# kylegrover/raymarch-algo-compare

Hardware: AMD Instinct MI355X
Metric: Mrays/sec (mean iters/ray alongside), 1920x1080 Mandelbulb/Standard (higher is better)
Workload: dtype f64

## Files before the change

### include/rm_hip.h

```cpp
#ifndef RM_HIP_H
#define RM_HIP_H

#include <stddef.h>
#include <stdint.h>

#ifdef __cplusplus
extern "C" {
#endif

#define RM_OK 0
#define RM_E_BAD_SCENE (-1)
#define RM_E_BAD_STRATEGY (-2)
#define RM_E_BAD_DIMS (-3)
#define RM_E_NO_DEVICE (-4)
#define RM_E_HIP (-5)
#define RM_E_BAD_ARG (-6)
#define RM_E_RCCL (-7)

#define RM_NUM_SCENES 20
#define RM_NUM_STRATEGIES 11
#define RM_NUM_STRATEGY_KERNELS 13
#define RM_HIST_BINS 544
#define RM_MAX_TIMED 256

// ... 48 lines not shown
    int32_t resume_grid;
    int32_t resume_mode;
    int32_t pipeline;
    int32_t team_grid;
    int32_t queue_first;
    int32_t team_steal;
    int32_t queue_refill_min;
    int32_t queue_retry;
    int32_t team_retry;
    int32_t age_priority;
    int32_t late_teams;
    int32_t exit_backlog;
    int32_t keep_busy;
    int32_t early_handover;
    int32_t early_trips;
    int32_t reserved1;
} RmFrameDesc;

typedef struct RmStats {
    uint64_t total_rays;
    uint64_t hit_count;
    uint64_t sum_iters;
    int32_t iter_max;
    int32_t iter_min;
    uint64_t iter_hist[RM_HIST_BINS];
    uint64_t sum_evals;
} RmStats;

typedef struct RmTiming {
    int32_t warmup;
    int32_t repeats;
// ... 238 lines not shown
```

### raymarch_algo_compare_amd/_native.py

```python
from __future__ import annotations

import ctypes
import os
import threading

import numpy as np

_HERE = os.path.dirname(os.path.abspath(__file__))
LIB_PATH = os.environ.get("RM_HIP_LIB") or os.path.join(_HERE, "librm_hip.so")

RM_NUM_SCENES = 20
RM_NUM_STRATEGIES = 11
RM_NUM_STRATEGY_KERNELS = 13
RM_HIST_BINS = 544
RM_MAX_TIMED = 256

ERROR_NAMES = {0: "RM_OK", -1: "RM_E_BAD_SCENE", -2: "RM_E_BAD_STRATEGY", -3: "RM_E_BAD_DIMS",
               -4: "RM_E_NO_DEVICE", -5: "RM_E_HIP", -6: "RM_E_BAD_ARG", -7: "RM_E_RCCL"}

EXPORTS = [
    "rm_init", "rm_shutdown", "rm_last_error", "rm_device_info", "rm_num_scenes", "rm_num_strategies",
    "rm_default_strategy_params",
    "rm_sdf_eval", "rm_march_rays", "rm_march_rays_team", "rm_render", "rm_render_outputs", "rm_render_device", "rm_stats_device_bytes",
    "rm_read_stats", "rm_bench_device", "rm_alloc_frame", "rm_free_frame", "rm_copy_frame_to_host",
# ... 75 lines not shown
    _fields_ = [("scene_id", ctypes.c_int32), ("strategy_id", ctypes.c_int32),
                ("width", ctypes.c_int32), ("height", ctypes.c_int32),
                ("row0", ctypes.c_int32), ("rows", ctypes.c_int32),
                ("cam", ctypes.c_double * 14), ("march", RmMarchConfig),
                ("tile_rows", ctypes.c_int32), ("refill_min", ctypes.c_int32),
                ("grid_waves", ctypes.c_int32), ("band_rows", ctypes.c_int32),
                ("band_stride", ctypes.c_int32), ("band_offset", ctypes.c_int32),
                ("tile_order_mode", ctypes.c_int32), ("eval_mode", ctypes.c_int32),
                ("suspend_after", ctypes.c_int32 * 2),
                ("resume_grid", ctypes.c_int32), ("resume_mode", ctypes.c_int32),
                ("pipeline", ctypes.c_int32), ("team_grid", ctypes.c_int32), ("queue_first", ctypes.c_int32),
                ("team_steal", ctypes.c_int32), ("queue_refill_min", ctypes.c_int32), ("queue_retry", ctypes.c_int32),
                ("team_retry", ctypes.c_int32), ("age_priority", ctypes.c_int32),
                ("late_teams", ctypes.c_int32), ("exit_backlog", ctypes.c_int32),
                ("keep_busy", ctypes.c_int32), ("early_handover", ctypes.c_int32),
                ("early_trips", ctypes.c_int32), ("reserved1", ctypes.c_int32)]


class RmOutputs(ctypes.Structure):
    _fields_ = [("depth", ctypes.c_void_p), ("iters", ctypes.c_void_p), ("hit", ctypes.c_void_p),
                ("t_raw", ctypes.c_void_p), ("final_sdf", ctypes.c_void_p), ("block_var", ctypes.c_void_p),
                ("evals", ctypes.c_void_p)]


class RmStats(ctypes.Structure):
    _fields_ = [("total_rays", ctypes.c_uint64), ("hit_count", ctypes.c_uint64),
                ("sum_iters", ctypes.c_uint64), ("iter_max", ctypes.c_int32), ("iter_min", ctypes.c_int32),
                ("iter_hist", ctypes.c_uint64 * RM_HIST_BINS), ("sum_evals", ctypes.c_uint64)]


class RmTiming(ctypes.Structure):
# ... 179 lines not shown

def device_info() -> dict:
    L = init()
    info = RmDeviceInfo()
    check(L.rm_device_info(ctypes.byref(info)))
    return {"name": info.name.decode(), "arch": info.arch.decode(), "device_id": info.device_id,
            "compute_units": info.compute_units, "clock_mhz": info.clock_mhz,
            "wavefront_size": info.wavefront_size, "total_mem_bytes": int(info.total_mem_bytes)}


def make_desc(scene_id, strategy_id, cam14, width, height, row0=0, rows=None, max_iterations=512,
              hit_threshold=1e-4, max_distance=100.0, lipschitz=1.0, full=False, tile_rows=0, refill_min=0,
              grid_waves=0, band_rows=0, band_stride=0, band_offset=0, tile_order_mode=0, eval_mode=0,
              suspend_after=(0, 0), resume_grid=0, resume_mode=0, params: dict | None = None, pipeline=0, team_grid=0,
              queue_first=0, team_steal=0, queue_refill_min=0, queue_retry=0, team_retry=0, age_priority=0, late_teams=0,
              exit_backlog=0, keep_busy=0, early_handover=0, early_trips=0) -> RmFrameDesc:
    d = RmFrameDesc()
    d.scene_id, d.strategy_id = int(scene_id), int(strategy_id)
    d.width, d.height = int(width), int(height)
    d.row0 = int(row0)
    d.rows = int(height - row0 if rows is None else rows)
    cam14 = np.asarray(cam14, dtype=np.float64).ravel()
    if cam14.size != 14:
        raise ValueError("cam14 must hold 14 doubles")
    for i in range(14):
        d.cam[i] = float(cam14[i])
    d.march.max_iterations = int(max_iterations)
    d.march.full = 1 if full else 0
    d.march.hit_threshold = float(hit_threshold)
    d.march.max_distance = float(max_distance)
    d.march.lipschitz = float(lipschitz)
    fill_params(d.march, params)
    d.tile_rows, d.refill_min, d.grid_waves = int(tile_rows), int(refill_min), int(grid_waves)
    d.band_rows, d.band_stride, d.band_offset = int(band_rows), int(band_stride), int(band_offset)
    d.tile_order_mode = int(tile_order_mode)
    d.eval_mode = int(eval_mode)
    d.suspend_after[0], d.suspend_after[1] = int(suspend_after[0]), int(suspend_after[1])
    d.resume_grid = int(resume_grid)
    d.resume_mode = int(resume_mode)
    d.pipeline, d.team_grid, d.queue_first, d.team_steal = int(pipeline), int(team_grid), int(queue_first), int(team_steal)
    d.queue_refill_min, d.queue_retry, d.team_retry = int(queue_refill_min), int(queue_retry), int(team_retry)
    d.age_priority = int(age_priority)
    d.late_teams, d.exit_backlog = int(late_teams), int(exit_backlog)
    d.keep_busy = int(keep_busy)
    d.early_handover = int(early_handover)
    d.early_trips = int(early_trips)
    return d


def _ptr(a):
    return None if a is None else a.ctypes.data_as(ctypes.c_void_p)


def _ref(record):
    return ctypes.byref(record) if record is not None else None


def _timing(warmup, repeats):
    if repeats <= 0:
        return None
    tm = RmTiming()
# ... 383 lines not shown
```

### raymarch_algo_compare_amd/csrc/rm_capi.hip

```cpp
#include <hip/hip_runtime.h>
#include <dlfcn.h>
#include <link.h>
#include <rccl/rccl.h>

#include <algorithm>
#include <cstdarg>
#include <cstdio>
#include <cstdlib>
#include <cstring>
#include <map>
#include <memory>
#include <mutex>
#include <optional>
#include <string>
#include <vector>

#include "../../include/rm_hip.h"
#include "rm_kernels.h"
#include "rm_launch_plan.h"
#include "rm_pipeline.h"
#include "rm_scene_program.h"
#include "rm_interval.h"
#include "rm_interval_catalogue.h"
#include "rm_segment.h"
// ... 125 lines not shown
    long long corder_key[12] = { -1 };
    bool corder_valid = false;
    bool pass_timing = false;
    hipEvent_t pev[RM_MAX_PASSES + 1];
    bool pev_ready = false;
    int pass_count = 0;
    bool last_was_pipeline = false;
    const unsigned long long* last_stats = nullptr;
    float long_marks[4] = { 0.f, 0.f, 0.f, 0.f };
    float last_push_ms = 0.f, last_pop_ms = 0.f;
    uint32_t generation = 0;
    struct QueueKey { int stride = 0; int writer = 0; size_t used = 0; } qkey[rm::kQueues];
    hipEvent_t frame_ev = nullptr;
    hipStream_t frame_stream = nullptr;
    bool frame_ev_valid = false;
};

struct State : Session {
    WsBuf stats, depth, iters, hit, traw, fs, bvar, evals, tcost, torder, queue[rm::kQueues];
    WsBuf in[2], out[4];
    WsBuf bstats;
    WsBuf ivprog;
    WsBuf ctl;
    WsBuf busy;
    WsBuf trace, trace_start, trace_detach;
    WsBuf ccost, corder;
    WsBuf ssim_depth, ssim_normal, ssim_color, ssim_hit;
    WsBuf ssim_ref, ssim_part, ssim_ssd, ssim_out;
    WsBuf score_depth, score_normal, score_hit, score_caps;
    WsBuf score_band, score_keys, score_small, score_part;
// ... 218 lines not shown
}

int check_desc(const RmFrameDesc* d)
{
    if (!d) return fail(RM_E_BAD_ARG, "desc is NULL");
    if (int rc = check_scene(d->scene_id)) return rc;
    if (d->strategy_id < 0 || d->strategy_id >= RM_NUM_STRATEGY_KERNELS)
        return fail(RM_E_BAD_STRATEGY, "strategy_id %d out of range", d->strategy_id);
    if (int rc = check_slice(d, d->band_rows > 0 && d->band_stride > 1)) return rc;
    if (d->tile_rows != 0 && d->tile_rows != 4 && d->tile_rows != 1) return fail(RM_E_BAD_ARG, "tile_rows must be 0, 4 or 1");
    if (d->tile_order_mode < 0 || d->tile_order_mode > 4) return fail(RM_E_BAD_ARG, "tile_order_mode must be 0 .. 4");
    if (d->eval_mode < 0 || d->eval_mode > 2) return fail(RM_E_BAD_ARG, "eval_mode must be 0, 1 or 2");
    if (d->resume_mode < 0 || d->resume_mode > 3) return fail(RM_E_BAD_ARG, "resume_mode must be 0..3");
    if (d->resume_grid < 0) return fail(RM_E_BAD_ARG, "negative resume_grid");
    if (d->pipeline < 0 || d->pipeline > 2) return fail(RM_E_BAD_ARG, "pipeline must be 0, 1 or 2");
    if (d->team_grid < 0 || d->queue_first < 0 || d->queue_first > 3 || d->team_steal < 0 || d->team_steal > 2 ||
        d->queue_refill_min < 0 || d->queue_refill_min > 64 || d->queue_retry < 0 || d->team_retry < 0 || d->age_priority < 0)
        return fail(RM_E_BAD_ARG, "bad single-launch tuning field");
    if (d->exit_backlog < 0 || d->late_teams > 65536) return fail(RM_E_BAD_ARG, "bad late-team field");
    if (d->keep_busy > (1 << 20)) return fail(RM_E_BAD_ARG, "keep_busy out of range");
    if (d->early_handover > (1 << 20)) return fail(RM_E_BAD_ARG, "early_handover out of range");
    if (d->early_trips < 0 || d->early_trips > 64) return fail(RM_E_BAD_ARG, "early_trips out of range");
    if (d->band_rows < 0 || d->band_stride < 0 || d->band_offset < 0) return fail(RM_E_BAD_ARG, "negative band parameter");
    if (d->band_rows > 0 && d->band_stride > 1) {
        const int th = d->tile_rows ? d->tile_rows : 4;
        if (d->band_rows % th) return fail(RM_E_BAD_ARG, "band_rows must be a multiple of the tile height %d", th);
        if (d->band_offset >= d->band_stride) return fail(RM_E_BAD_ARG, "band_offset must be < band_stride");
        if (d->rows > 0) {
            const long long y = d->rows - 1;
            const long long last = d->row0 + ((y / d->band_rows) * d->band_stride + d->band_offset) * d->band_rows + y % d->band_rows;
// ... 174 lines not shown
}

int launch_frame(const RmFrameDesc* d, const rm::LaunchPlan& p, rm::KernelArgs a, hipStream_t s);

int launch(const RmFrameDesc* d, const rm::LaunchPlan& p, const rm::KernelArgs& a, hipStream_t s)
{
    if (g.frame_ev_valid && g.frame_stream != s) HIP_TRY(hipStreamWaitEvent(s, g.frame_ev, 0));
    const int rc_frame = launch_frame(d, p, a, s);
    if (rc_frame) return rc_frame;
    if (!g.frame_ev_valid) {
        HIP_TRY(hipEventCreateWithFlags(&g.frame_ev, hipEventDisableTiming));
        g.frame_ev_valid = true;
    }
    HIP_TRY(hipEventRecord(g.frame_ev, s));
    g.frame_stream = s;
    return RM_OK;
}

int launch_frame(const RmFrameDesc* d, const rm::LaunchPlan& p, rm::KernelArgs a, hipStream_t s)
{
    a.raw_outputs = (a.t_raw || a.final_sdf || a.evals) ? 1 : 0;
    const bool own_stats = a.stats == (unsigned long long*)g.stats.p;
    if (!(own_stats && g.stats_ready)) HIP_TRY(hipMemsetAsync(a.stats, 0, kStatsBytes, s));
    if (own_stats) g.stats_ready = a.fused_reduce != 0;
    if (d->rows == 0) return RM_OK;
    if (p.refuse) return fail(RM_E_BAD_ARG, "%s", p.refuse);
    const rm::SceneLaunchers* const sc = launchers(d->scene_id);
    const int ntiles = a.tiles_per_frame * a.nframes;
    int order = p.tile_order;
    if (order == 1) {
// ... 78 lines not shown
            const size_t npix = (size_t)a.rows * a.width * a.nframes;
            int rc3;
            if ((rc3 = g.trace.ensure((8 + 8 * kTraceRecords) * 4)) || (rc3 = g.trace_start.ensure(npix * 4)) ||
                (rc3 = g.trace_detach.ensure(npix * 4)))
                return rc3;
            HIP_TRY(hipMemsetAsync(g.trace.p, 0, 32, s));
            HIP_TRY(hipMemsetAsync(g.trace_start.p, 0, npix * 4, s));
            HIP_TRY(hipMemsetAsync(g.trace_detach.p, 0, npix * 4, s));
            a.trace = (uint32_t*)g.trace.p;
            a.trace_cap = (uint32_t)kTraceRecords;
            a.trace_start = (uint32_t*)g.trace_start.p;
            a.trace_detach = (uint32_t*)g.trace_detach.p;
            g.trace_pix = npix;
        }
        if (a.tile_cost) HIP_TRY(hipMemsetAsync(a.tile_cost, 0, (size_t)ntiles * 4, s));
        HIP_TRY(sc->pipeline(d->strategy_id, a, p.pipeline_grid, s));
        if (pt) HIP_TRY(hipEventRecord(g.pev[++g.pass_count], s));
        g.last_was_pipeline = true;
        g.last_stats = a.stats;
    } else {
        HIP_TRY(sc->render(d->strategy_id, a, p.render_grid, s));
        if (pt) HIP_TRY(hipEventRecord(g.pev[++g.pass_count], s));
    }
    if (p.park[0] > 0 && !p.single) {
        rm::KernelArgs b = a;
        b.suspend_after = p.park[1];
        b.suspend_queue = 1;
        b.refill_min = p.resume_refill_min;
        b.team_wgs = p.resume_grid;
        b.keep_busy = p.pass_keep_busy;
        if (p.pass_team[0])
// ... 298 lines not shown
        return fail(RM_E_NO_DEVICE, "device %d is %s; this library carries gfx950 code only", device_id, g.prop.gcnArchName);
    HIP_TRY(hipStreamCreateWithFlags(&g.stream, hipStreamNonBlocking));
    int rc = g.stats.ensure(kStatsBytes);
    if (rc) return rc;
    g.device = device_id;
    g.ready = true;
    return RM_OK;
}

void rm_shutdown(void)
{
    std::lock_guard<std::mutex> lk(g_mu);
    if (!g.ready) return;
    (void)hipSetDevice(g.device);
    (void)hipStreamSynchronize(g.stream);
    g_seen_streams.clear();
    release_all(g_workspace_bufs);
    if (g.frame_ev_valid) (void)hipEventDestroy(g.frame_ev);
    if (g.events) for (auto& e : g.ev) (void)hipEventDestroy(e);
    if (g.pev_ready) for (auto& e : g.pev) (void)hipEventDestroy(e);
    {
        std::lock_guard<std::mutex> lp(g_prog_mu);
        for (auto& kv : g_programs)
            if (kv.second.dev) {
                (void)hipFree(kv.second.dev);
                kv.second.dev = nullptr;
            }
    }
    (void)hipStreamDestroy(g.stream);
    static_cast<Session&>(g) = Session();
// ... 1207 lines not shown
```

### raymarch_algo_compare_amd/csrc/rm_kernels.h

```cpp
#pragma once

#define RM_TABLES_IN_LDS 1

#include <hip/hip_runtime.h>
#include <stdint.h>
#include <type_traits>

#include "rm_camera.h"
#include "rm_capture.h"
#include "rm_scenes.h"
#include "rm_shape.h"
#include "rm_strategies.h"

namespace rm {

constexpr int kHistBins = 544;
constexpr int kStatsHead = 24;
constexpr int kStatsWords = kStatsHead + kHistBins;
constexpr int kQueues = 2;
constexpr int kStatsParts = 64;
constexpr int kStatsBlocks = 1 + kStatsParts;

struct FrameParams {
    CameraParams cam;
// ... 978 lines not shown
struct SceneLaunchers {
    hipError_t (*render)(int strategy, const KernelArgs& a, int grid, hipStream_t s);
    hipError_t (*resume)(int strategy, int level, const KernelArgs& a, int grid, hipStream_t s);
    hipError_t (*resume_team)(int strategy, int level, const KernelArgs& a, int grid, hipStream_t s);
    hipError_t (*pipeline)(int strategy, const KernelArgs& a, int grid, hipStream_t s);
    hipError_t (*occupancy_pipeline)(int strategy, int interleave, int batch, int* blocks_per_cu);
    bool has_teams;
    int (*entry_bytes)(int strategy);
    hipError_t (*occupancy)(int strategy, int interleave, int batch, int* blocks_per_cu);
    hipError_t (*sdf_eval)(const double* xyz, size_t n, double* out, const void* scene_data, hipStream_t s);
    hipError_t (*march_rays)(int strategy, const MarchCfg& cfg, const double* o, const double* d, size_t n,
                             uint8_t* hit, double* t, int32_t* iters, double* fs, const void* scene_data, hipStream_t s);
    hipError_t (*march_rays_team)(int strategy, const MarchCfg& cfg, const double* o, const double* d, size_t n,
                                  uint8_t* hit, double* t, int32_t* iters, double* fs, unsigned long long* busy, int fillers, hipStream_t s);
    hipError_t (*capture)(const CaptureArgs& a, int nframes, hipStream_t s);
};

}
```

### raymarch_algo_compare_amd/csrc/rm_pipeline.h

```cpp
#pragma once

#include "rm_kernels.h"

namespace rm {

constexpr int kCtlStride = 16;
constexpr int kCTile = 0;
constexpr int kCReserved = 1;
constexpr int kCTaken = 3;
constexpr int kCFreshDone = 5;
constexpr int kCProdExited = 6;
constexpr int kCLeft = 7;
constexpr int kCLateStarted = 8;
constexpr int kCTeamDone = 9;
constexpr int kCtlWords = 10 * kCtlStride;
__device__ __forceinline__ unsigned long long* ctl(const KernelArgs& a, int k) { return a.ctl + k * kCtlStride; }
constexpr int kWMarkStart = 13;
constexpr int kWMarkFresh = 14;
constexpr int kWMarkProd = 15;
constexpr int kWMarkTiles = 17;
constexpr int kWMarkPush = 18;
constexpr int kWMarkPop = 19;
constexpr int kWLongPushMax = 20;
constexpr int kWLongTeamMax = 21;
// ... 154 lines not shown
        const uint32_t y = pix / (uint32_t)a.width, x = pix - y * (uint32_t)a.width;
        atomicMax(&a.tile_cost[frame * (uint32_t)a.tiles_per_frame + (y / (uint32_t)a.tile_h) * (uint32_t)a.tiles_x + (x >> 6)], it);
    }
}

template <class Scene, class E>
__device__ __forceinline__ auto early_handover(const KernelArgs& a, const E& ev, int i) -> decltype(Scene::eval_trips(ev), bool())
{
    return a.early_handover > 0 && i >= a.early_handover && Scene::eval_trips(ev) >= a.early_trips;
}
template <class Scene>
__device__ __forceinline__ bool early_handover(const KernelArgs&, const NoEval&, int) { return false; }
template <class Scene, class E>
__device__ __forceinline__ bool early_handover(const KernelArgs&, const E&, long) { return false; }

template <class Scene, class Strat, int TILE_H, bool INTERLEAVE, bool BATCH>
__global__ __launch_bounds__(64 * kPipeWaves, 2) void pipeline_kernel(const KernelArgs a)
{
    static_assert(!INTERLEAVE || SceneIterative<Scene>::value, "INTERLEAVE needs Scene::Eval");
    constexpr bool TEAMS = SceneIterative<Scene>::value;
    constexpr int TILE_PIX = kTileW * TILE_H;
    using Entry = QEntry<Strat>;
    using PLds = PipeProducerLds<TILE_PIX>;
    constexpr size_t kRoleBytes = sizeof(PLds) > sizeof(PipeTeamLds) ? sizeof(PLds) : sizeof(PipeTeamLds);
    __shared__ __attribute__((aligned(16))) unsigned char s_role[kRoleBytes];
    __shared__ unsigned int s_hist[kHistBins];
    __shared__ unsigned int s_leave;

    const int lane = lane_id();
    const int wave = (int)(threadIdx.x >> 6);
    for (int b = threadIdx.x; b < kHistBins; b += blockDim.x) s_hist[b] = 0u;
    if (threadIdx.x == 0) s_leave = 0u;
    rm_load_tables<Scene>();
    __syncthreads();
    if (a.marks && threadIdx.x == 0) atomicMax(&a.stats[kWMarkStart], ~realtime());

    WaveAcc acc;
    const bool late_team = TEAMS && (int)blockIdx.x >= a.late_team_first;
    const bool team_wg = TEAMS && ((int)blockIdx.x < a.team_wgs || late_team);
    if (late_team && threadIdx.x == 0) __hip_atomic_fetch_add(ctl(a, kCLateStarted), 1ull, __ATOMIC_RELAXED, __HIP_MEMORY_SCOPE_AGENT);
    constexpr int kRole[8] = { 0, 1, 2, -1, -1, -1, -1, -1 };
    const int wave_role = !team_wg ? -2 : kRole[wave & 7];
    const bool team_role = team_wg && wave_role >= 0;
    if (team_wg) {
        PipeTeamLds& T = *reinterpret_cast<PipeTeamLds*>(s_role);
        for (int b = threadIdx.x; b < kHistBins; b += blockDim.x) T.hist[b] = 0u;
        if (threadIdx.x == 0) { T.base = T.count = T.queue = T.done = 0u; T.ok_lo = T.ok_hi = 0u; }
        __syncthreads();
    }

    if constexpr (TEAMS) {
    if (team_wg && wave_role == -1) return;
    if (team_role) {
        if (a.team_prio >= 3) __builtin_amdgcn_s_setprio(3);
        else if (a.team_prio == 2) __builtin_amdgcn_s_setprio(2);
        else if (a.team_prio == 1) __builtin_amdgcn_s_setprio(1);
        const int team = wave_role / kTeam;
        PipeTeamLds& L = reinterpret_cast<PipeTeamLds*>(s_role)[team];
        const int part = wave_role % kTeam;
        bool active = false;
        uint32_t my_gi = 0;
        uint32_t my_push = 0;
        uint32_t my_pop = 0, nev_pop = 0;
        int nev = 0;
        vec3 origin = v3(0.0, 0.0, 0.0), dir = v3(0.0, 0.0, 0.0);
        MarchCfg lane_cfg = a.single.cfg;
        if constexpr (!BATCH) pin_cfg(lane_cfg);
        const MarchCfg& cfg = lane_cfg;
        Strat s;
        typename Scene::Eval ev;
        int turn = 0;
        int since_try = 0;
        unsigned long long idle_since = 0;

        for (;;) {
            const unsigned long long idle = __ballot(!active);
            const int nidle = __popcll(idle);
            const bool look = nidle == 64 || (nidle >= a.refill_min && since_try >= a.team_retry);
            if (look) {
                since_try = 0;
                if (part == 0) {
                    unsigned int base = 0, done = 0;
                    int q = 1, cnt = 0;
                    if (lane == 0) {
                        cnt = q_claim_lane0(a, 1, nidle, base);
                        if (cnt == 0 && a.team_steal) { q = 0; cnt = q_claim_lane0(a, 0, nidle, base); }
                        if (cnt == 0 && nidle == 64) {
                            const unsigned long long ex = ld_relaxed(ctl(a, kCProdExited));
                            if (ex >= (unsigned long long)a.producer_waves && q_available(a, 1) <= 0 && q_available(a, 0) <= 0) done = 1;
                            const unsigned long long now = realtime();
                            if (idle_since == 0) idle_since = now;
                            if (!done && now - idle_since > kMaxTeamWaitTicks) { atomicMax(&a.stats[kWError], 2ull); done = 1; }
                        } else if (cnt > 0) {
                            idle_since = 0;
                            if (a.marks && q == 1) atomicMax(&a.stats[kWMarkPop], realtime());
                        }
                    }
                    cnt = __builtin_amdgcn_readfirstlane(cnt);
                    q = __builtin_amdgcn_readfirstlane(q);
                    base = (unsigned int)__builtin_amdgcn_readfirstlane((int)base);
                    unsigned long long okm = 0;
                    if (cnt > 0) {
                        const int rank = rank_in_mask(idle);
                        const bool want = !active && rank < cnt;
                        const bool got = q_wait_ready<Strat>(a, q, want, base + (unsigned int)rank);
                        okm = __ballot(want && got);
                    }
                    if (lane == 0) {
                        L.base = base; L.count = (unsigned int)cnt; L.queue = (unsigned int)q; L.done = done;
                        L.ok_lo = (unsigned int)okm; L.ok_hi = (unsigned int)(okm >> 32);
                    }
                }
                __syncthreads();
                const unsigned int base = L.base, cnt = L.count, q = L.queue, done = L.done;
                const unsigned long long okm = ((unsigned long long)L.ok_hi << 32) | (unsigned long long)L.ok_lo;
                __syncthreads();
                if (done) break;
                if (cnt > 0) {
                    if (part != 0) __builtin_amdgcn_fence(__ATOMIC_ACQUIRE, "agent");
                    const int rank = rank_in_mask(idle);
                    const bool mine = ((okm >> lane) & 1ull) != 0;
                    if (mine) {
                        const Entry* const e = (const Entry*)a.queue[q] + (base + (unsigned int)rank);
                        my_gi = e->gi;
                        nev = (int)e->nev;
                        s = e->s;
                        my_push = e->pad;
                        if (a.trace) { my_pop = (uint32_t)(realtime() - ~ld_relaxed(&a.stats[kWMarkStart])); nev_pop = (uint32_t)nev; }
                        uint32_t frame; int x, gy;
                        element_pixel(a, my_gi, frame, x, gy);
                        if constexpr (BATCH) {
                            const FrameParams& fp = a.frames[frame];
                            camera_ray(fp.cam, a.width, a.height, x, gy, origin, dir);
                            lane_cfg = fp.cfg;
                            lane_cfg.full = a.full;
                        } else {
                            camera_ray(a.single.cam, a.width, a.height, x, gy, origin, dir);
                        }
                        active = true;
                    }
                } else if (nidle == 64) {
                    __builtin_amdgcn_s_sleep(127);
                    __builtin_amdgcn_s_sleep(127);
                    continue;
                }
            }
            if (!__any(active)) continue;

            ++since_try;
            bool ready = true;
            if (active) ready = Scene::begin(ev, origin + dir * s.te);
            team_trips<Scene>(part, ready, [&](auto P, bool go) { return team_trip<Scene>(ev, go, P, lane, L.xch, turn); });
            const int live = a.trace ? __popcll(__ballot(active)) : 0;
            if (active) {
                ++nev;
                if (s.step(Scene::value(ev), cfg)) {
                    active = false;
                    if (part == 0) {
                        store_direct(a, my_gi, s.res, nev, acc, L.hist);
                        if (a.trace) {
                            const uint32_t k = atomicAdd(&a.trace[0], 1u);
                            if (k < a.trace_cap) {
                                uint32_t* const r = a.trace + 8 + 8 * (size_t)k;
                                r[0] = my_gi; r[1] = (uint32_t)s.res.iters; r[2] = my_push; r[3] = my_pop;
                                r[4] = (uint32_t)(realtime() - ~ld_relaxed(&a.stats[kWMarkStart]));
                                r[5] = nev_pop; r[6] = (uint32_t)nev; r[7] = (uint32_t)blockIdx.x | ((uint32_t)live << 16);
                            }
                        }
                        if (a.marks && s.res.iters >= kLongRay) {
                            const unsigned long long now = realtime() - ~ld_relaxed(&a.stats[kWMarkStart]);
                            atomicMax(&a.stats[kWLongPushMax], (unsigned long long)my_push);
                            atomicMax(&a.stats[kWLongPushMin], ~(unsigned long long)my_push);
                            atomicMax(&a.stats[kWLongTeamMax], now - my_push);
                            atomicMax(&a.stats[kWLongTeamMin], ~(now - my_push));
                        }
                    }
                }
            }
        }
        unsigned long long* const spart = stats_part(a.stats);
        if (part == 0) acc.flush(spart);
        __syncthreads();
        for (int b = part * 64 + lane; b < kHistBins; b += 64 * kTeam) {
            const unsigned int c = L.hist[b];
            if (c) atomicAdd(&spart[kStatsHead + b], (unsigned long long)c);
        }
        if (part == 0 && lane == 0) __hip_atomic_fetch_add(ctl(a, kCTeamDone), 1ull, __ATOMIC_RELAXED, __HIP_MEMORY_SCOPE_AGENT);
        return;
    }
    }

    PLds& L = *reinterpret_cast<PLds*>(s_role);
    float (*const s_depth)[TILE_PIX] = L.depth[wave];
    uint32_t (*const s_ih)[TILE_PIX] = L.ih[wave];
    const int ntiles = a.tiles_per_frame * a.nframes;
    const int team_wgs = TEAMS ? a.team_wgs : 0;
    const int pwave = ((int)blockIdx.x - team_wgs) * kPipeWaves + wave;
    const int park0 = a.suspend_after;
    const int park1 = (TEAMS && a.team_wgs > 0) ? a.suspend_after2 : 0;
    const bool queues = park0 > 0;
    const bool detach = a.q0_detach != 0;
    const bool may_leave = TEAMS && detach && park1 > 0 && ((int)blockIdx.x - team_wgs) < a.early_exit_wgs;
    bool leaving = false;

    int slot_tile[kSlots], slot_out[kSlots];
#pragma unroll
    for (int k = 0; k < kSlots; ++k) { slot_tile[k] = -1; slot_out[k] = 0; }
    int cur = 0;
    int pool_next = TILE_PIX;
    bool more_tiles = true;
    bool first_tile = true;
    TileGeom cg = { 0, 0, 0, 0, 0, 0, 0 };

    bool active = false;
    bool resumed = false;
    bool nopark = false;
    int my_slot = 0, my_pix = 0;
// ... 328 lines not shown
    unsigned long long* const part = stats_part(a.stats);
    acc.flush(part);
    if (queues && lane == 0) {
        if (!fresh_reported) add_after_drain(ctl(a, kCFreshDone), 1ull);
        add_after_drain(ctl(a, kCProdExited), 1ull);
        if (a.marks) atomicMax(&a.stats[kWMarkProd], realtime());
    }
    __syncthreads();
    for (int b = threadIdx.x; b < kHistBins; b += blockDim.x) {
        const unsigned int c = s_hist[b];
        if (c) atomicAdd(&part[kStatsHead + b], (unsigned long long)c);
    }
    if (TEAMS && a.keep_busy > 0 && !team_wg && a.team_wgs > 0) keep_busy_until(ctl(a, kCTeamDone), (unsigned long long)a.team_wgs, a.keep_busy);
}

}
```

### raymarch_algo_compare_amd/csrc/rm_scene_tu.hip

```cpp
#include "rm_kernels.h"
#if defined(RM_SCENE_PROGRAM)
#include "rm_scene_program.h"
#else
#include "rm_pipeline.h"
#endif

#if !defined(RM_SCENE_ID) && !defined(RM_SCENE_PROGRAM)
#error "compile with -DRM_SCENE_ID=<scene id> or -DRM_SCENE_PROGRAM"
#endif

namespace rm {

#if defined(RM_SCENE_PROGRAM_EXT)
using SceneT = SceneExtProgram;
#elif defined(RM_SCENE_PROGRAM)
using SceneT = SceneProgram;
#else
template <int ID> struct SceneById;
#define RM_X(id, S) template <> struct SceneById<id> { using type = S; };
RM_SCENE_LIST(RM_X)
#undef RM_X
using SceneT = SceneById<RM_SCENE_ID>::type;
#endif

// ... 75 lines not shown
    return blocks_per_cu(render_fn(strategy, interleave, batch), 64 * kWavesPerWG, blocks);
}

static hipError_t resume(int strategy, int level, const KernelArgs& a, int grid, hipStream_t s)
{
    return launch(resume_fn(strategy, a.interleave, a.frames != nullptr), grid, 64 * kWavesPerWG, s, a, level);
}

static hipError_t resume_team(int strategy, int level, const KernelArgs& a, int grid, hipStream_t s)
{
    return launch(resume_team_fn(strategy, a.frames != nullptr), grid, 64 * kTeam, s, a, level);
}

#if defined(RM_SCENE_PROGRAM)
#define RM_PIPELINE_FNS nullptr, nullptr
#else
#define RM_PIPELINE_FNS pipeline, occupancy_pipeline
static FrameKernel pipeline_fn(int strategy, int tile_h, int interleave, int batch)
{
    return with_strategy(strategy, FrameKernel(), [&](auto t) -> FrameKernel {
        using S = typename decltype(t)::type;
        if constexpr (kIter) {
            if (tile_h == 1)
                return with_mode(interleave, batch, [](auto il, auto b) -> FrameKernel { return pipeline_kernel<SceneT, S, 1, il(), b()>; });
        }
        if (tile_h != 4) return nullptr;
        return with_mode(interleave, batch, [](auto il, auto b) -> FrameKernel { return pipeline_kernel<SceneT, S, 4, il(), b()>; });
    });
}

static hipError_t pipeline(int strategy, const KernelArgs& a, int grid, hipStream_t s)
{
    return launch(pipeline_fn(strategy, a.tile_h, a.interleave, a.frames != nullptr), grid, 64 * kPipeWaves, s, a);
}

static hipError_t occupancy_pipeline(int strategy, int interleave, int batch, int* blocks)
{
    return blocks_per_cu(pipeline_fn(strategy, 4, interleave, batch), 64 * kPipeWaves, blocks);
}
#endif

static int entry_bytes(int strategy)
{
    return with_strategy(strategy, 0, [](auto t) { return (int)sizeof(QEntry<typename decltype(t)::type>); });
}

static hipError_t sdf_eval(const double* xyz, size_t n, double* out, const void* scene_data, hipStream_t s)
{
    if (n == 0) return hipSuccess;
    return launch(sdf_eval_kernel<SceneT>, (int)((n + 255) / 256), 256, s, xyz, n, out, scene_data);
}

static hipError_t march_rays(int strategy, const MarchCfg& cfg, const double* o, const double* d, size_t n,
                             uint8_t* hit, double* t, int32_t* iters, double* fs, const void* scene_data, hipStream_t s)
// ... 30 lines not shown
#if defined(RM_SCENE_PROGRAM)
static_assert(!kIter, "a scene program has no resumable evaluation");
#if defined(RM_SCENE_PROGRAM_EXT)
#define RM_LAUNCHERS_FN scene_launchers_program_ext
#else
#define RM_LAUNCHERS_FN scene_launchers_program
#endif
#else
#define RM_CAT2(a, b) a##b
#define RM_CAT(a, b) RM_CAT2(a, b)
#define RM_LAUNCHERS_FN RM_CAT(scene_launchers_, RM_SCENE_ID)
#endif
const SceneLaunchers* RM_LAUNCHERS_FN()
{
    static const SceneLaunchers l = { render, resume, kIter ? resume_team : nullptr, RM_PIPELINE_FNS, kIter,
                                      entry_bytes, occupancy, sdf_eval, march_rays, kIter ? march_rays_team : nullptr, capture };
    return &l;
}

}
```

Measured before the change: 272.6.

## Split fused pipeline into separate producer and team kernels on concurrent streams

Splits the single persistent pipeline launch, whose workgroups take either a producer or a team role, into two kernels. The producer kernel is specialised without team code, and a smaller team kernel sized for 64*kTeam threads runs on a second non-blocking stream, with events to join the streams. Each kernel can use fewer registers and less LDS than the fused version. When both split kernels reach the fused kernel's occupancy, the split form is chosen by default. The cost is extra launch and event overhead, plus reliance on both kernels actually being co-resident for the queue handoff to progress.

```diff
diff --git a/include/rm_hip.h b/include/rm_hip.h
--- a/include/rm_hip.h
+++ b/include/rm_hip.h
@@ -86,7 +86,7 @@
     int32_t keep_busy;
     int32_t early_handover;
     int32_t early_trips;
-    int32_t reserved1;
+    int32_t pipeline_form;
 } RmFrameDesc;
 
 typedef struct RmStats {
diff --git a/raymarch_algo_compare_amd/_native.py b/raymarch_algo_compare_amd/_native.py
--- a/raymarch_algo_compare_amd/_native.py
+++ b/raymarch_algo_compare_amd/_native.py
@@ -113,7 +113,7 @@
                 ("team_retry", ctypes.c_int32), ("age_priority", ctypes.c_int32),
                 ("late_teams", ctypes.c_int32), ("exit_backlog", ctypes.c_int32),
                 ("keep_busy", ctypes.c_int32), ("early_handover", ctypes.c_int32),
-                ("early_trips", ctypes.c_int32), ("reserved1", ctypes.c_int32)]
+                ("early_trips", ctypes.c_int32), ("pipeline_form", ctypes.c_int32)]
 
 
 class RmOutputs(ctypes.Structure):
@@ -323,7 +323,7 @@
               grid_waves=0, band_rows=0, band_stride=0, band_offset=0, tile_order_mode=0, eval_mode=0,
               suspend_after=(0, 0), resume_grid=0, resume_mode=0, params: dict | None = None, pipeline=0, team_grid=0,
               queue_first=0, team_steal=0, queue_refill_min=0, queue_retry=0, team_retry=0, age_priority=0, late_teams=0,
-              exit_backlog=0, keep_busy=0, early_handover=0, early_trips=0) -> RmFrameDesc:
+              exit_backlog=0, keep_busy=0, early_handover=0, early_trips=0, pipeline_form=0) -> RmFrameDesc:
     d = RmFrameDesc()
     d.scene_id, d.strategy_id = int(scene_id), int(strategy_id)
     d.width, d.height = int(width), int(height)
@@ -354,6 +354,7 @@
     d.keep_busy = int(keep_busy)
     d.early_handover = int(early_handover)
     d.early_trips = int(early_trips)
+    d.pipeline_form = int(pipeline_form)
     return d
 
 
diff --git a/raymarch_algo_compare_amd/csrc/rm_capi.hip b/raymarch_algo_compare_amd/csrc/rm_capi.hip
--- a/raymarch_algo_compare_amd/csrc/rm_capi.hip
+++ b/raymarch_algo_compare_amd/csrc/rm_capi.hip
@@ -163,6 +163,8 @@
     hipEvent_t frame_ev = nullptr;
     hipStream_t frame_stream = nullptr;
     bool frame_ev_valid = false;
+    hipStream_t team_stream = nullptr;
+    hipEvent_t split_ev[2] = { nullptr, nullptr };
 };
 
 struct State : Session {
@@ -411,6 +413,7 @@
     if (d->resume_mode < 0 || d->resume_mode > 3) return fail(RM_E_BAD_ARG, "resume_mode must be 0..3");
     if (d->resume_grid < 0) return fail(RM_E_BAD_ARG, "negative resume_grid");
     if (d->pipeline < 0 || d->pipeline > 2) return fail(RM_E_BAD_ARG, "pipeline must be 0, 1 or 2");
+    if (d->pipeline_form < 0 || d->pipeline_form > 3) return fail(RM_E_BAD_ARG, "pipeline_form must be 0 .. 3");
     if (d->team_grid < 0 || d->queue_first < 0 || d->queue_first > 3 || d->team_steal < 0 || d->team_steal > 2 ||
         d->queue_refill_min < 0 || d->queue_refill_min > 64 || d->queue_retry < 0 || d->team_retry < 0 || d->age_priority < 0)
         return fail(RM_E_BAD_ARG, "bad single-launch tuning field");
@@ -615,6 +618,33 @@
     }
     HIP_TRY(hipEventRecord(g.frame_ev, s));
     g.frame_stream = s;
+    return RM_OK;
+}
+
+#ifndef RM_SPLIT_BY_DEFAULT
+#define RM_SPLIT_BY_DEFAULT 1
+#endif
+constexpr bool kSplitByDefault = RM_SPLIT_BY_DEFAULT != 0;
+int single_launch_form(const RmFrameDesc* d, const rm::LaunchPlan& p, const rm::KernelArgs& a, const rm::SceneLaunchers* sc, int* form)
+{
+    *form = 1;
+    if (d->pipeline_form == 1) return RM_OK;
+    const bool covered = sc->pipeline_teams && sc->pipeline_producers && p.team_wgs > 0 && p.suspend_after2 > 0 && p.q0_detach != 0 &&
+                         p.early_exit_wgs == 0 && p.late_team_first == p.pipeline_grid;
+    if (d->pipeline_form >= 2) {
+        if (!covered)
+            return fail(RM_E_BAD_ARG, "pipeline_form %d: the split form exists for single launches with teams in detach mode without late teams", d->pipeline_form);
+        *form = d->pipeline_form;
+        return RM_OK;
+    }
+    if (!kSplitByDefault || !covered || a.frames) return RM_OK;
+    if (d->strategy_id == 7 || d->strategy_id == 9) return RM_OK;
+    int fused = 0, producers = 0, teams = 0;
+    if (sc->occupancy_pipeline(d->strategy_id, a.interleave, 0, &fused) != hipSuccess ||
+        sc->occupancy_split(d->strategy_id, a.tile_h, a.interleave, 0, &producers, &teams) != hipSuccess)
+        return RM_OK;
+    const int per_cu = rm::grid_per_cu(fused);
+    if (producers >= per_cu && teams >= per_cu) *form = 2;
     return RM_OK;
 }
 
@@ -723,7 +753,29 @@
             g.trace_pix = npix;
         }
         if (a.tile_cost) HIP_TRY(hipMemsetAsync(a.tile_cost, 0, (size_t)ntiles * 4, s));
-        HIP_TRY(sc->pipeline(d->strategy_id, a, p.pipeline_grid, s));
+        int form = 1;
+        if (int rcf = single_launch_form(d, p, a, sc, &form)) return rcf;
+        if (form == 1) {
+            HIP_TRY(sc->pipeline(d->strategy_id, a, p.pipeline_grid, s));
+        } else {
+            const int producer_wgs = p.pipeline_grid - p.team_wgs;
+            hipStream_t ts = s;
+            if (form == 2) {
+                if (!g.team_stream) {
+                    HIP_TRY(hipStreamCreateWithFlags(&g.team_stream, hipStreamNonBlocking));
+                    for (auto& e : g.split_ev) HIP_TRY(hipEventCreateWithFlags(&e, hipEventDisableTiming));
+                }
+                ts = g.team_stream;
+                HIP_TRY(hipEventRecord(g.split_ev[0], s));
+                HIP_TRY(hipStreamWaitEvent(ts, g.split_ev[0], 0));
+            }
+            HIP_TRY(sc->pipeline_producers(d->strategy_id, a, producer_wgs, s));
+            HIP_TRY(sc->pipeline_teams(d->strategy_id, a, p.team_wgs, ts));
+            if (form == 2) {
+                HIP_TRY(hipEventRecord(g.split_ev[1], ts));
+                HIP_TRY(hipStreamWaitEvent(s, g.split_ev[1], 0));
+            }
+        }
         if (pt) HIP_TRY(hipEventRecord(g.pev[++g.pass_count], s));
         g.last_was_pipeline = true;
         g.last_stats = a.stats;
@@ -1052,6 +1104,16 @@
     if (!g.ready) return;
     (void)hipSetDevice(g.device);
     (void)hipStreamSynchronize(g.stream);
+    if (g.team_stream) {
+        (void)hipStreamSynchronize(g.team_stream);
+        for (auto& e : g.split_ev) (void)hipEventDestroy(e);
+        (void)hipStreamDestroy(g.team_stream);
+    }
+    for (void* s : g_own_streams) {
+        (void)hipStreamSynchronize((hipStream_t)s);
+        (void)hipStreamDestroy((hipStream_t)s);
+    }
+    g_own_streams.clear();
     g_seen_streams.clear();
     release_all(g_workspace_bufs);
     if (g.frame_ev_valid) (void)hipEventDestroy(g.frame_ev);
diff --git a/raymarch_algo_compare_amd/csrc/rm_kernels.h b/raymarch_algo_compare_amd/csrc/rm_kernels.h
--- a/raymarch_algo_compare_amd/csrc/rm_kernels.h
+++ b/raymarch_algo_compare_amd/csrc/rm_kernels.h
@@ -1016,6 +1016,9 @@
     hipError_t (*march_rays_team)(int strategy, const MarchCfg& cfg, const double* o, const double* d, size_t n,
                                   uint8_t* hit, double* t, int32_t* iters, double* fs, unsigned long long* busy, int fillers, hipStream_t s);
     hipError_t (*capture)(const CaptureArgs& a, int nframes, hipStream_t s);
+    hipError_t (*pipeline_producers)(int strategy, const KernelArgs& a, int grid, hipStream_t s);
+    hipError_t (*pipeline_teams)(int strategy, const KernelArgs& a, int grid, hipStream_t s);
+    hipError_t (*occupancy_split)(int strategy, int tile_h, int interleave, int batch, int* producers_per_cu, int* teams_per_cu);
 };
 
 }
diff --git a/raymarch_algo_compare_amd/csrc/rm_pipeline.h b/raymarch_algo_compare_amd/csrc/rm_pipeline.h
--- a/raymarch_algo_compare_amd/csrc/rm_pipeline.h
+++ b/raymarch_algo_compare_amd/csrc/rm_pipeline.h
@@ -192,15 +192,153 @@
 template <class Scene, class E>
 __device__ __forceinline__ bool early_handover(const KernelArgs&, const E&, long) { return false; }
 
-template <class Scene, class Strat, int TILE_H, bool INTERLEAVE, bool BATCH>
-__global__ __launch_bounds__(64 * kPipeWaves, 2) void pipeline_kernel(const KernelArgs a)
+template <class Scene, class Strat, bool BATCH>
+__device__ __forceinline__ void pipe_team_role(const KernelArgs& a, const KernelArgs& ar, PipeTeamLds& L, const int part, const int lane)
+{
+    WaveAcc acc;
+    if (a.team_prio >= 3) __builtin_amdgcn_s_setprio(3);
+    else if (a.team_prio == 2) __builtin_amdgcn_s_setprio(2);
+    else if (a.team_prio == 1) __builtin_amdgcn_s_setprio(1);
+    bool active = false;
+    uint32_t my_gi = 0;
+    uint32_t my_push = 0;
+    uint32_t my_pop = 0, nev_pop = 0;
+    int nev = 0;
+    vec3 origin = v3(0.0, 0.0, 0.0), dir = v3(0.0, 0.0, 0.0);
+    MarchCfg lane_cfg = a.single.cfg;
+    if constexpr (!BATCH) pin_cfg(lane_cfg);
+    const MarchCfg& cfg = lane_cfg;
+    Strat s;
+    typename Scene::Eval ev;
+    int turn = 0;
+    int since_try = 0;
+    unsigned long long idle_since = 0;
+
+    for (;;) {
+        const unsigned long long idle = __ballot(!active);
+        const int nidle = __popcll(idle);
+        const bool look = nidle == 64 || (nidle >= a.refill_min && since_try >= a.team_retry);
+        if (look) {
+            since_try = 0;
+            if (part == 0) {
+                unsigned int base = 0, done = 0;
+                int q = 1, cnt = 0;
+                if (lane == 0) {
+                    cnt = q_claim_lane0(ar, 1, nidle, base);
+                    if (cnt == 0 && ar.team_steal) { q = 0; cnt = q_claim_lane0(ar, 0, nidle, base); }
+                    if (cnt == 0 && nidle == 64) {
+                        const unsigned long long ex = ld_relaxed(ctl(ar, kCProdExited));
+                        if (ex >= (unsigned long long)ar.producer_waves && q_available(ar, 1) <= 0 && q_available(ar, 0) <= 0) done = 1;
+                        const unsigned long long now = realtime();
+                        if (idle_since == 0) idle_since = now;
+                        if (!done && now - idle_since > kMaxTeamWaitTicks) { atomicMax(&ar.stats[kWError], 2ull); done = 1; }
+                    } else if (cnt > 0) {
+                        idle_since = 0;
+                        if (ar.marks && q == 1) atomicMax(&ar.stats[kWMarkPop], realtime());
+                    }
+                }
+                cnt = __builtin_amdgcn_readfirstlane(cnt);
+                q = __builtin_amdgcn_readfirstlane(q);
+                base = (unsigned int)__builtin_amdgcn_readfirstlane((int)base);
+                unsigned long long okm = 0;
+                if (cnt > 0) {
+                    const int rank = rank_in_mask(idle);
+                    const bool want = !active && rank < cnt;
+                    const bool got = q_wait_ready<Strat>(ar, q, want, base + (unsigned int)rank);
+                    okm = __ballot(want && got);
+                }
+                if (lane == 0) {
+                    L.base = base; L.count = (unsigned int)cnt; L.queue = (unsigned int)q; L.done = done;
+                    L.ok_lo = (unsigned int)okm; L.ok_hi = (unsigned int)(okm >> 32);
+                }
+            }
+            __syncthreads();
+            const unsigned int base = L.base, cnt = L.count, q = L.queue, done = L.done;
+            const unsigned long long okm = ((unsigned long long)L.ok_hi << 32) | (unsigned long long)L.ok_lo;
+            __syncthreads();
+            if (done) break;
+            if (cnt > 0) {
+                if (part != 0) __builtin_amdgcn_fence(__ATOMIC_ACQUIRE, "agent");
+                const int rank = rank_in_mask(idle);
+                const bool mine = ((okm >> lane) & 1ull) != 0;
+                if (mine) {
+                    const QEntry<Strat>* const e = (const QEntry<Strat>*)ar.queue[q] + (base + (unsigned int)rank);
+                    my_gi = e->gi;
+                    nev = (int)e->nev;
+                    s = e->s;
+                    my_push = e->pad;
+                    if (ar.trace) { my_pop = (uint32_t)(realtime() - ~ld_relaxed(&ar.stats[kWMarkStart])); nev_pop = (uint32_t)nev; }
+                    uint32_t frame; int x, gy;
+                    element_pixel(ar, my_gi, frame, x, gy);
+                    if constexpr (BATCH) {
+                        const FrameParams& fp = ar.frames[frame];
+                        camera_ray(fp.cam, ar.width, ar.height, x, gy, origin, dir);
+                        lane_cfg = fp.cfg;
+                        lane_cfg.full = ar.full;
+                    } else {
+                        camera_ray(ar.single.cam, ar.width, ar.height, x, gy, origin, dir);
+                    }
+                    active = true;
+                }
+            } else if (nidle == 64) {
+                __builtin_amdgcn_s_sleep(127);
+                __builtin_amdgcn_s_sleep(127);
+                continue;
+            }
+        }
+        if (!__any(active)) continue;
+
+        ++since_try;
+        bool ready = true;
+        if (active) ready = Scene::begin(ev, origin + dir * s.te);
+        team_trips<Scene>(part, ready, [&](auto P, bool go) { return team_trip<Scene>(ev, go, P, lane, L.xch, turn); });
+        const int live = a.trace ? __popcll(__ballot(active)) : 0;
+        if (active) {
+            ++nev;
+            if (s.step(Scene::value(ev), cfg)) {
+                active = false;
+                if (part == 0) {
+                    store_direct(ar, my_gi, s.res, nev, acc, L.hist);
+                    if (ar.trace) {
+                        const uint32_t k = atomicAdd(&ar.trace[0], 1u);
+                        if (k < ar.trace_cap) {
+                            uint32_t* const r = ar.trace + 8 + 8 * (size_t)k;
+                            r[0] = my_gi; r[1] = (uint32_t)s.res.iters; r[2] = my_push; r[3] = my_pop;
+                            r[4] = (uint32_t)(realtime() - ~ld_relaxed(&ar.stats[kWMarkStart]));
+                            r[5] = nev_pop; r[6] = (uint32_t)nev; r[7] = (uint32_t)blockIdx.x | ((uint32_t)live << 16);
+                        }
+                    }
+                    if (ar.marks && s.res.iters >= kLongRay) {
+                        const unsigned long long now = realtime() - ~ld_relaxed(&ar.stats[kWMarkStart]);
+                        atomicMax(&ar.stats[kWLongPushMax], (unsigned long long)my_push);
+                        atomicMax(&ar.stats[kWLongPushMin], ~(unsigned long long)my_push);
+                        atomicMax(&ar.stats[kWLongTeamMax], now - my_push);
+                        atomicMax(&ar.stats[kWLongTeamMin], ~(now - my_push));
+                    }
+                }
+            }
+        }
+    }
+    unsigned long long* const spart = stats_part(ar.stats);
+    if (part == 0) acc.flush(spart);
+    __syncthreads();
+    for (int b = part * 64 + lane; b < kHistBins; b += 64 * kTeam) {
+        const unsigned int c = L.hist[b];
+        if (c) atomicAdd(&spart[kStatsHead + b], (unsigned long long)c);
+    }
+    if (part == 0 && lane == 0) __hip_atomic_fetch_add(ctl(ar, kCTeamDone), 1ull, __ATOMIC_RELAXED, __HIP_MEMORY_SCOPE_AGENT);
+}
+
+template <class Scene, class Strat, int TILE_H, bool INTERLEAVE, bool BATCH, bool TEAM_ROLE, bool SPLIT>
+__device__ __forceinline__ void pipeline_body(const KernelArgs& ka, const KernelArgs& a)
 {
     static_assert(!INTERLEAVE || SceneIterative<Scene>::value, "INTERLEAVE needs Scene::Eval");
     constexpr bool TEAMS = SceneIterative<Scene>::value;
+    static_assert(TEAMS || !TEAM_ROLE, "team workgroups need a team form");
     constexpr int TILE_PIX = kTileW * TILE_H;
     using Entry = QEntry<Strat>;
     using PLds = PipeProducerLds<TILE_PIX>;
-    constexpr size_t kRoleBytes = sizeof(PLds) > sizeof(PipeTeamLds) ? sizeof(PLds) : sizeof(PipeTeamLds);
+    constexpr size_t kRoleBytes = (!TEAM_ROLE || sizeof(PLds) > sizeof(PipeTeamLds)) ? sizeof(PLds) : sizeof(PipeTeamLds);
     __shared__ __attribute__((aligned(16))) unsigned char s_role[kRoleBytes];
     __shared__ unsigned int s_hist[kHistBins];
     __shared__ unsigned int s_leave;
@@ -214,8 +352,8 @@
     if (a.marks && threadIdx.x == 0) atomicMax(&a.stats[kWMarkStart], ~realtime());
 
     WaveAcc acc;
-    const bool late_team = TEAMS && (int)blockIdx.x >= a.late_team_first;
-    const bool team_wg = TEAMS && ((int)blockIdx.x < a.team_wgs || late_team);
+    const bool late_team = TEAM_ROLE && (int)blockIdx.x >= a.late_team_first;
+    const bool team_wg = TEAM_ROLE && ((int)blockIdx.x < a.team_wgs || late_team);
     if (late_team && threadIdx.x == 0) __hip_atomic_fetch_add(ctl(a, kCLateStarted), 1ull, __ATOMIC_RELAXED, __HIP_MEMORY_SCOPE_AGENT);
     constexpr int kRole[8] = { 0, 1, 2, -1, -1, -1, -1, -1 };
     const int wave_role = !team_wg ? -2 : kRole[wave & 7];
@@ -227,143 +365,12 @@
         __syncthreads();
     }
 
-    if constexpr (TEAMS) {
+    if constexpr (TEAM_ROLE) {
     if (team_wg && wave_role == -1) return;
     if (team_role) {
-        if (a.team_prio >= 3) __builtin_amdgcn_s_setprio(3);
-        else if (a.team_prio == 2) __builtin_amdgcn_s_setprio(2);
-        else if (a.team_prio == 1) __builtin_amdgcn_s_setprio(1);
         const int team = wave_role / kTeam;
-        PipeTeamLds& L = reinterpret_cast<PipeTeamLds*>(s_role)[team];
         const int part = wave_role % kTeam;
-        bool active = false;
-        uint32_t my_gi = 0;
-        uint32_t my_push = 0;
-        uint32_t my_pop = 0, nev_pop = 0;
-        int nev = 0;
-        vec3 origin = v3(0.0, 0.0, 0.0), dir = v3(0.0, 0.0, 0.0);
-        MarchCfg lane_cfg = a.single.cfg;
-        if constexpr (!BATCH) pin_cfg(lane_cfg);
-        const MarchCfg& cfg = lane_cfg;
-        Strat s;
-        typename Scene::Eval ev;
-        int turn = 0;
-        int since_try = 0;
-        unsigned long long idle_since = 0;
-
-        for (;;) {
-            const unsigned long long idle = __ballot(!active);
-            const int nidle = __popcll(idle);
-            const bool look = nidle == 64 || (nidle >= a.refill_min && since_try >= a.team_retry);
-            if (look) {
-                since_try = 0;
-                if (part == 0) {
-                    unsigned int base = 0, done = 0;
-                    int q = 1, cnt = 0;
-                    if (lane == 0) {
-                        cnt = q_claim_lane0(a, 1, nidle, base);
-                        if (cnt == 0 && a.team_steal) { q = 0; cnt = q_claim_lane0(a, 0, nidle, base); }
-                        if (cnt == 0 && nidle == 64) {
-                            const unsigned long long ex = ld_relaxed(ctl(a, kCProdExited));
-                            if (ex >= (unsigned long long)a.producer_waves && q_available(a, 1) <= 0 && q_available(a, 0) <= 0) done = 1;
-                            const unsigned long long now = realtime();
-                            if (idle_since == 0) idle_since = now;
-                            if (!done && now - idle_since > kMaxTeamWaitTicks) { atomicMax(&a.stats[kWError], 2ull); done = 1; }
-                        } else if (cnt > 0) {
-                            idle_since = 0;
-                            if (a.marks && q == 1) atomicMax(&a.stats[kWMarkPop], realtime());
-                        }
-                    }
-                    cnt = __builtin_amdgcn_readfirstlane(cnt);
-                    q = __builtin_amdgcn_readfirstlane(q);
-                    base = (unsigned int)__builtin_amdgcn_readfirstlane((int)base);
-                    unsigned long long okm = 0;
-                    if (cnt > 0) {
-                        const int rank = rank_in_mask(idle);
-                        const bool want = !active && rank < cnt;
-                        const bool got = q_wait_ready<Strat>(a, q, want, base + (unsigned int)rank);
-                        okm = __ballot(want && got);
-                    }
-                    if (lane == 0) {
-                        L.base = base; L.count = (unsigned int)cnt; L.queue = (unsigned int)q; L.done = done;
-                        L.ok_lo = (unsigned int)okm; L.ok_hi = (unsigned int)(okm >> 32);
-                    }
-                }
-                __syncthreads();
-                const unsigned int base = L.base, cnt = L.count, q = L.queue, done = L.done;
-                const unsigned long long okm = ((unsigned long long)L.ok_hi << 32) | (unsigned long long)L.ok_lo;
-                __syncthreads();
-                if (done) break;
-                if (cnt > 0) {
-                    if (part != 0) __builtin_amdgcn_fence(__ATOMIC_ACQUIRE, "agent");
-                    const int rank = rank_in_mask(idle);
-                    const bool mine = ((okm >> lane) & 1ull) != 0;
-                    if (mine) {
-                        const Entry* const e = (const Entry*)a.queue[q] + (base + (unsigned int)rank);
-                        my_gi = e->gi;
-                        nev = (int)e->nev;
-                        s = e->s;
-                        my_push = e->pad;
-                        if (a.trace) { my_pop = (uint32_t)(realtime() - ~ld_relaxed(&a.stats[kWMarkStart])); nev_pop = (uint32_t)nev; }
-                        uint32_t frame; int x, gy;
-                        element_pixel(a, my_gi, frame, x, gy);
-                        if constexpr (BATCH) {
-                            const FrameParams& fp = a.frames[frame];
-                            camera_ray(fp.cam, a.width, a.height, x, gy, origin, dir);
-                            lane_cfg = fp.cfg;
-                            lane_cfg.full = a.full;
-                        } else {
-                            camera_ray(a.single.cam, a.width, a.height, x, gy, origin, dir);
-                        }
-                        active = true;
-                    }
-                } else if (nidle == 64) {
-                    __builtin_amdgcn_s_sleep(127);
-                    __builtin_amdgcn_s_sleep(127);
-                    continue;
-                }
-            }
-            if (!__any(active)) continue;
-
-            ++since_try;
-            bool ready = true;
-            if (active) ready = Scene::begin(ev, origin + dir * s.te);
-            team_trips<Scene>(part, ready, [&](auto P, bool go) { return team_trip<Scene>(ev, go, P, lane, L.xch, turn); });
-            const int live = a.trace ? __popcll(__ballot(active)) : 0;
-            if (active) {
-                ++nev;
-                if (s.step(Scene::value(ev), cfg)) {
-                    active = false;
-                    if (part == 0) {
-                        store_direct(a, my_gi, s.res, nev, acc, L.hist);
-                        if (a.trace) {
-                            const uint32_t k = atomicAdd(&a.trace[0], 1u);
-                            if (k < a.trace_cap) {
-                                uint32_t* const r = a.trace + 8 + 8 * (size_t)k;
-                                r[0] = my_gi; r[1] = (uint32_t)s.res.iters; r[2] = my_push; r[3] = my_pop;
-                                r[4] = (uint32_t)(realtime() - ~ld_relaxed(&a.stats[kWMarkStart]));
-                                r[5] = nev_pop; r[6] = (uint32_t)nev; r[7] = (uint32_t)blockIdx.x | ((uint32_t)live << 16);
-                            }
-                        }
-                        if (a.marks && s.res.iters >= kLongRay) {
-                            const unsigned long long now = realtime() - ~ld_relaxed(&a.stats[kWMarkStart]);
-                            atomicMax(&a.stats[kWLongPushMax], (unsigned long long)my_push);
-                            atomicMax(&a.stats[kWLongPushMin], ~(unsigned long long)my_push);
-                            atomicMax(&a.stats[kWLongTeamMax], now - my_push);
-                            atomicMax(&a.stats[kWLongTeamMin], ~(now - my_push));
-                        }
-                    }
-                }
-            }
-        }
-        unsigned long long* const spart = stats_part(a.stats);
-        if (part == 0) acc.flush(spart);
-        __syncthreads();
-        for (int b = part * 64 + lane; b < kHistBins; b += 64 * kTeam) {
-            const unsigned int c = L.hist[b];
-            if (c) atomicAdd(&spart[kStatsHead + b], (unsigned long long)c);
-        }
-        if (part == 0 && lane == 0) __hip_atomic_fetch_add(ctl(a, kCTeamDone), 1ull, __ATOMIC_RELAXED, __HIP_MEMORY_SCOPE_AGENT);
+        pipe_team_role<Scene, Strat, BATCH>(a, a, reinterpret_cast<PipeTeamLds*>(s_role)[team], part, lane);
         return;
     }
     }
@@ -371,14 +378,15 @@
     PLds& L = *reinterpret_cast<PLds*>(s_role);
     float (*const s_depth)[TILE_PIX] = L.depth[wave];
     uint32_t (*const s_ih)[TILE_PIX] = L.ih[wave];
-    const int ntiles = a.tiles_per_frame * a.nframes;
-    const int team_wgs = TEAMS ? a.team_wgs : 0;
-    const int pwave = ((int)blockIdx.x - team_wgs) * kPipeWaves + wave;
-    const int park0 = a.suspend_after;
-    const int park1 = (TEAMS && a.team_wgs > 0) ? a.suspend_after2 : 0;
+    const int ntiles = ka.tiles_per_frame * ka.nframes;
+    const int team_wgs = TEAM_ROLE ? a.team_wgs : 0;
+    int pwave = ((int)blockIdx.x - team_wgs) * kPipeWaves + wave;
+    if constexpr (SPLIT) pwave = __builtin_amdgcn_readfirstlane(pwave);
+    const int park0 = ka.suspend_after;
+    const int park1 = (TEAMS && ka.team_wgs > 0) ? ka.suspend_after2 : 0;
     const bool queues = park0 > 0;
-    const bool detach = a.q0_detach != 0;
-    const bool may_leave = TEAMS && detach && park1 > 0 && ((int)blockIdx.x - team_wgs) < a.early_exit_wgs;
+    const bool detach = SPLIT || a.q0_detach != 0;
+    const bool may_leave = !SPLIT && TEAMS && detach && park1 > 0 && ((int)blockIdx.x - team_wgs) < a.early_exit_wgs;
     bool leaving = false;
 
     int slot_tile[kSlots], slot_out[kSlots];
@@ -737,4 +745,32 @@
     if (TEAMS && a.keep_busy > 0 && !team_wg && a.team_wgs > 0) keep_busy_until(ctl(a, kCTeamDone), (unsigned long long)a.team_wgs, a.keep_busy);
 }
 
-}
+template <class Scene, class Strat, int TILE_H, bool INTERLEAVE, bool BATCH>
+__global__ __launch_bounds__(64 * kPipeWaves, 2) void pipeline_kernel(const KernelArgs a)
+{
+    pipeline_body<Scene, Strat, TILE_H, INTERLEAVE, BATCH, SceneIterative<Scene>::value, false>(a, a);
+}
+
+template <class Scene, class Strat, int TILE_H, bool INTERLEAVE, bool BATCH>
+__global__ __launch_bounds__(64 * kPipeWaves, 2) void pipeline_producer_kernel(const KernelArgs a)
+{
+    __shared__ KernelArgs s_args;
+    if (threadIdx.x == 0) s_args = a;
+    pipeline_body<Scene, Strat, TILE_H, INTERLEAVE, BATCH, false, true>(a, s_args);
+}
+
+template <class Scene, class Strat, bool BATCH>
+__global__ __launch_bounds__(64 * kTeam) void pipeline_team_kernel(const KernelArgs a)
+{
+    __shared__ PipeTeamLds T;
+    __shared__ KernelArgs s_args;
+    if (threadIdx.x == 0) s_args = a;
+    for (int b = threadIdx.x; b < kHistBins; b += blockDim.x) T.hist[b] = 0u;
+    if (threadIdx.x == 0) { T.base = T.count = T.queue = T.done = 0u; T.ok_lo = T.ok_hi = 0u; }
+    rm_load_tables<Scene>();
+    __syncthreads();
+    if (a.marks && threadIdx.x == 0) atomicMax(&a.stats[kWMarkStart], ~realtime());
+    pipe_team_role<Scene, Strat, BATCH>(a, s_args, T, (int)(threadIdx.x >> 6), lane_id());
+}
+
+}
diff --git a/raymarch_algo_compare_amd/csrc/rm_scene_tu.hip b/raymarch_algo_compare_amd/csrc/rm_scene_tu.hip
--- a/raymarch_algo_compare_amd/csrc/rm_scene_tu.hip
+++ b/raymarch_algo_compare_amd/csrc/rm_scene_tu.hip
@@ -113,6 +113,7 @@
 
 #if defined(RM_SCENE_PROGRAM)
 #define RM_PIPELINE_FNS nullptr, nullptr
+#define RM_SPLIT_FNS nullptr, nullptr, nullptr
 #else
 #define RM_PIPELINE_FNS pipeline, occupancy_pipeline
 static FrameKernel pipeline_fn(int strategy, int tile_h, int interleave, int batch)
@@ -137,6 +138,46 @@
 {
     return blocks_per_cu(pipeline_fn(strategy, 4, interleave, batch), 64 * kPipeWaves, blocks);
 }
+
+static FrameKernel pipeline_producer_fn(int strategy, int tile_h, int interleave, int batch)
+{
+    return with_strategy(strategy, FrameKernel(), [&](auto t) -> FrameKernel {
+        using S = typename decltype(t)::type;
+        if constexpr (kIter) {
+            if (tile_h == 1)
+                return with_mode(interleave, batch, [](auto il, auto b) -> FrameKernel { return pipeline_producer_kernel<SceneT, S, 1, il(), b()>; });
+            if (tile_h == 4)
+                return with_mode(interleave, batch, [](auto il, auto b) -> FrameKernel { return pipeline_producer_kernel<SceneT, S, 4, il(), b()>; });
+        }
+        return nullptr;
+    });
+}
+
+static FrameKernel pipeline_team_fn(int strategy, int batch)
+{
+    return with_strategy(strategy, FrameKernel(), [&](auto t) -> FrameKernel {
+        using S = typename decltype(t)::type;
+        if constexpr (kIter) return batch ? pipeline_team_kernel<SceneT, S, true> : pipeline_team_kernel<SceneT, S, false>;
+        return nullptr;
+    });
+}
+
+static hipError_t pipeline_producers(int strategy, const KernelArgs& a, int grid, hipStream_t s)
+{
+    return launch(pipeline_producer_fn(strategy, a.tile_h, a.interleave, a.frames != nullptr), grid, 64 * kPipeWaves, s, a);
+}
+
+static hipError_t pipeline_teams(int strategy, const KernelArgs& a, int grid, hipStream_t s)
+{
+    return launch(pipeline_team_fn(strategy, a.frames != nullptr), grid, 64 * kTeam, s, a);
+}
+
+static hipError_t occupancy_split(int strategy, int tile_h, int interleave, int batch, int* producers, int* teams)
+{
+    const hipError_t e = blocks_per_cu(pipeline_producer_fn(strategy, tile_h, interleave, batch), 64 * kPipeWaves, producers);
+    return e != hipSuccess ? e : blocks_per_cu(pipeline_team_fn(strategy, batch), 64 * kTeam, teams);
+}
+#define RM_SPLIT_FNS (kIter ? pipeline_producers : nullptr), (kIter ? pipeline_teams : nullptr), (kIter ? occupancy_split : nullptr)
 #endif
 
 static int entry_bytes(int strategy)
@@ -197,7 +238,8 @@
 const SceneLaunchers* RM_LAUNCHERS_FN()
 {
     static const SceneLaunchers l = { render, resume, kIter ? resume_team : nullptr, RM_PIPELINE_FNS, kIter,
-                                      entry_bytes, occupancy, sdf_eval, march_rays, kIter ? march_rays_team : nullptr, capture };
+                                      entry_bytes, occupancy, sdf_eval, march_rays, kIter ? march_rays_team : nullptr, capture,
+                                      RM_SPLIT_FNS };
     return &l;
 }
 
```

Measured after the change: 278.4, median of 6. 1.02x the previous value.
